# wolfecameron/GIST

Hardware: AMD Instinct MI355X
Metric: epochs/sec (higher is better)
Workload: dtype f32 (projection products from 3 bf16 pieces per operand = all 24 bits, 6 cross terms, fp32 accumulation)

## Files before the change

### gist_amd/_lib.py

```python
import ctypes
import os

_HERE = os.path.dirname(os.path.abspath(__file__))
LIB_PATH = os.environ.get('GIST_LIB_PATH') or os.path.join(_HERE, 'libgist_hip.so')

ABI_VERSION = 16


class GistLibraryError(RuntimeError):
    pass


class GistError(RuntimeError):
    """A gist_* entry point returned a negative code."""


_p = ctypes.c_void_p
_i64 = ctypes.c_int64
_i32 = ctypes.c_int32
_int = ctypes.c_int
_f = ctypes.c_float
_u64 = ctypes.c_uint64

SIGNATURES = {
    'gist_last_error': (ctypes.c_char_p, []),
    'gist_abi_version': (_int, []),
    'gist_device_count': (_int, []),
    'gist_in_degree_norm_f32': (_int, [_p, _i64, _p, _p]),
    'gist_spmm_csr_f32': (_int, [_p, _p, _p, _i64, _p, _i64, _i64, _i64, _p, _p, _int, _p]),
    'gist_partition_last_stats': (_int, [_p, _i32]),
    'gist_partition_graph': (_int, [_p, _p, _p, _p, _i64, _i32, _u64, _i32, _f, _p]),
    'gist_spmm_csr_blocked_f32': (_int, [_p, _p, _p, _i64, _p, _i64, _i64, _i64, _p, _p, _int, _p, _i64, _p]),
    'gist_spmm_blocks_bytes': (_i64, [_i64]),
    'gist_spmm_blocks_prepare': (_int, [_p, _p, _i64, _p, _i64, _p, _i64, _p]),
    'gist_spmm_csr_prepared_f32': (_int, [_p, _p, _p, _i64, _p, _i64, _i64, _i64, _p, _p, _int, _p, _i64, _p, _p]),
    'gist_gemm_workspace_bytes': (_i64, [_i64, _i64, _i64]),
    'gist_gemm_set_mode': (_int, [_int]),
    'gist_gemm_get_mode': (_int, []),
    'gist_tuning_set': (_int, [_int, ctypes.c_double]),
    'gist_tuning_get': (ctypes.c_double, [_int]),
    'gist_launch_count': (ctypes.c_uint64, []),
    'gist_empty_launches': (_int, [ctypes.c_int32, ctypes.c_int32, ctypes.c_int32, _p]),
    'gist_gemm_nt_f32': (_int, [_p, _i64, _p, _i64, _p, _p, _i64, _i64, _i64, _i64, _p, _i64, _p]),
    'gist_gemm_nn_f32': (_int, [_p, _i64, _p, _i64, _p, _i64, _i64, _i64, _i64, _p, _i64, _p]),
    'gist_gemm_tn_f32': (_int, [_p, _i64, _p, _i64, _p, _i64, _i64, _i64, _i64, _p, _i64, _p]),
    'gist_ln_relu_fwd_f32': (_int, [_p, _i64, _p, _i64, _p, _i64, _i64, _int, _int, _f, _p]),
    'gist_ln_relu_bwd_f32': (_int, [_p, _i64, _p, _i64, _p, _p, _i64, _i64, _i64, _int, _int, _p]),
    'gist_gemm_nn_dropout_f32': (_int, [_p, _i64, _p, _i64, _p, _i64, _i64, _i64, _i64, _f, _u64, _u64, _p, _i64, _p]),
    'gist_dropout_f32': (_int, [_p, _i64, _i64, _i64, _f, _u64, _u64, _p]),
    'gist_colsum_partials': (_i64, [_i64]),
    'gist_colsum_f32': (_int, [_p, _i64, _i64, _i64, _p, _p, _p]),
    'gist_softmax_xent_f32': (_int, [_p, _i64, _p, _p, _i64, _p, _p, _p, _i64, _i64, _i64, _p]),
    'gist_adam_f32': (_int, [_p, _p, _p, _p, _i64, _f, _f, _f, _f, _f, _i64, _p]),
    'gist_argmax_correct_i32': (_int, [_p, _i64, _p, _p, _p, _i64, _i64, _p]),
    'gist_induced_mark': (_int, [_p, _i64, _p, _p]),
    'gist_induced_unmark': (_int, [_p, _i64, _p, _p]),
    'gist_fill_i32': (_int, [_p, _i64, _i32, _p]),
    'gist_copy_i32': (_int, [_p, _p, _i64, _p]),
    'gist_publish_i64': (_int, [_p, _i64, _p, _p]),
    'gist_induced_rowptr': (_int, [_p, _p, _p, _i64, _p, _p, _p]),
    'gist_induced_fill': (_int, [_p, _p, _p, _i64, _p, _p, _p, _i64, _p]),
    'gist_extract_batch': (_int, [_p, _p, _p, _p, _p, _i64, _p, _p, _p, _p, _p, _i64, _p, _p, _i64, _i64, _p, _i64, _p, _p, _p]),
    'gist_gather_rows_f32': (_int, [_p, _i64, _p, _i64, _i64, _p, _i64, _p]),
    'gist_gather_i32': (_int, [_p, _p, _i64, _p, _p]),
    'gist_block_gather_f32': (_int, [_p, _i64, _p, _p, _i64, _i64, _p, _i64, _p]),
    'gist_block_scatter_f32': (_int, [_p, _i64, _p, _p, _i64, _i64, _p, _i64, _p]),
    'gist_mean_rows_f32': (_int, [_p, _i64, _i64, _i64, _p, _p]),
    'gist_standard_scaler_workspace_bytes': (_i64, [_i64, _i64]),
    'gist_standard_scaler_f32': (_int, [_p, _i64, _i64, _i64, _p, _i64, _p, _p, _p, _i64, _p]),
    'gist_timer_create': (_p, [_i64]),
    'gist_timer_destroy': (None, [_p]),
    'gist_timer_reset': (None, [_p]),
    'gist_timer_count': (_i64, [_p]),
    'gist_timer_read': (_int, [_p, _i64, _p, _p, _p, _p, _p]),
    'gist_step_h3_workspace_bytes': (_i64, [_p]),
    'gist_step_h3_workspace_bytes_mode': (_i64, [_p, _int]),
    'gist_step_fused_workspace_bytes': (_i64, [_p]),
    'gist_step_col_partials_floats': (_i64, [_p]),
    'gist_step_fused_slab_bytes': (_i64, [_p, _i32]),
    'gist_spmm_csr_drop_f32': (_int, [_p, _p, _p, _i64, _p, _i64, _i64, _i64, _p, _p, _int, _p, _i64, _int, _f,
                                      _u64, _u64, _u64, _i64, _p]),
    'gist_spmm_csr_drop_prepared_f32': (_int, [_p, _p, _p, _i64, _p, _i64, _i64, _i64, _p, _p, _int, _p, _i64, _int, _f,
                                               _u64, _u64, _u64, _i64, _p, _p]),
    'gist_spmm_csr_drop_lnbwd_f32': (_int, [_p, _p, _p, _i64, _p, _i64, _i64, _i64, _p, _p, _i64, _f, _u64, _u64, _u64, _i64,
                                            _p, _i64, _p, _p, _i64, _p, _i64, _int, _p]),
    'gist_spmm_lnb_units': (_i64, [_i64]),
    'gist_spmm_block_image_bytes': (_i64, []),
    'gist_spmm_pair_min_edges': (ctypes.c_int32, []),
    'gist_spmm_block_units_f32': (_int, [_p, _i64, _p, _p, _i64, _p, _i64, _i64, _i64, _p, _int, _p]),
    'gist_spmm_block_chains_f32': (_int, [_p, _i64, _p, _p, _p, _i64, _p, _i64, _i64, _i64, _p, _int, _p]),
    'gist_spmm_prepared_useful': (_int, [_i64, _i64, _i64, _p, _p]),
    'gist_spmm_drop_takes': (_int, [_int, _i64, _i64, _i64, _p, _p, _int]),
    'gist_gemm_dual_takes': (_int, [_i64, _i64, _i64, _i64, _i64, _i64, _i64, _p, _p, _p, _p]),
    'gist_gemm_nn_tn_dual_f32': (_int, [_p, _i64, _p, _i64, _p, _i64, _p, _i64, _p, _i64, _i64, _i64, _i64, _p, _i64, _p, _p]),
    'gist_gemm_slabs_f32': (_int, [_int, _p, _i64, _p, _i64, _p, _p, _i64, _i64, _i64, _i64, _p, _i64, _p, _p]),
    'gist_ln_relu_fwd_drop_f32': (_int, [_p, _i64, _p, _i64, _p, _i64, _p, _i64, _i64, _int, _int, _f, _f, _u64,
                                         _u64, _i64, _p]),
    'gist_ln_relu_fwd_slabs_f32': (_int, [_p, _i64, _p, _i64, _int, _p, _p, _i64, _p, _i64, _p, _i64, _i64, _int, _int,
                                          _f, _f, _u64, _u64, _i64, _p]),
    'gist_gemm_splits_operands': (_int, [_i64, _i64, _i64]),
    'gist_row_chunks16': (_i64, [_i64]),
    'gist_ln_relu_bwd_colsum_f32': (_int, [_p, _i64, _p, _i64, _p, _p, _i64, _i64, _i64, _int, _int, _p, _p]),
    'gist_colsum_chunks_f32': (_int, [_p, _i64, _i64, _p, _p]),
    'gist_class_layer_takes': (_int, [_i64, _i64, _i64, _i64, _i64, _p, _p]),
    'gist_class_layer_f32': (_int, [_p, _i64, _p, _i64, _p, _p, _i64, _p, _i64, _p, _i64, _p, _p, _i64, _f, _u64, _u64,
                                    _p, _i64, _i64, _i64, _p]),
    'gist_class_dw_slab_bytes': (_i64, [_i64, _i64, _i64]),
    'gist_class_dw_slabs_f32': (_int, [_p, _i64, _p, _i64, _p, _i64, _p, _i64, _i64, _i64, _p]),
    'gist_ln_relu_bwd_colsum_class_dw_f32': (_int, [_p, _i64, _p, _i64, _p, _p, _i64, _i64, _i64, _int, _int, _p,
                                                    _p, _i64, _p, _i64, _p, _i64, _p, _i64, _i64, _i64, _p]),
    'gist_gemm_nn_dropout_colsum_f32': (_int, [_p, _i64, _p, _i64, _p, _i64, _i64, _i64, _i64, _f, _u64, _u64,
                                               _p, _i64, _p, _p]),
    'gist_softmax_xent_slabs_f32': (_int, [_p, _i64, _p, _i64, _i64, _p, _p, _p, _i64, _p, _p, _p, _i64, _i64,
                                           _i64, _p]),
    'gist_adam_segments_f32': (_int, [_p, _p, _p, _p, _i64, _f, _f, _f, _f, _f, _i64, _p, _i64, _p, _i64, _i64,
                                      _p, _p]),
    'gist_grad_segments_finish_f32': (_int, [_p, _i64, _p, _i64, _p]),
    'gist_extract_batch_drop': (_int, [_p, _p, _p, _p, _p, _i64, _p, _p, _p, _p, _p, _i64, _p, _p, _i64, _i64, _p,
                                       _i64, _p, _p, _p, _i64, _f, _u64, _u64, _i64, _p]),
    'gist_extract_parts_scratch_bytes': (_i64, [_i64]),
    'gist_extract_parts_supported': (_int, [_i64]),
    'gist_extract_parts_batch': (_int, [_p, _p, _p, _p, _p, _i64, _i64, _p, _p, _i32, _p, _p, _p, _p, _i64,
                                        _p, _p, _i64, _i64, _p, _i64, _p, _p, _p, _i64, _f, _u64, _u64, _i64, _p,
                                        _p]),
    'gist_sage_step': (_int, [_p, _p, _i64, _u64, _f, _f, _f, _f, _f, _i64, _int, _p]),
    'gist_sage_step_extracts_next': (_int, [_p, _i64, _int]),
    'gist_extract_parts_desc_batch': (_int, [_p, _p]),
    'gist_adam_segments_extract_f32': (_int, [_p, _p, _p, _p, _i64, _f, _f, _f, _f, _f, _i64, _p, _i64, _p, _i64, _i64,
                                              _p, _p, _p]),
}

GIST_MAX_LAYERS = 16
TUNE = {'h3_min_gflop': 0, 'h3_min_tiles': 1, 'h3_tm': 2, 'gemm_tile': 3, 'gemm_splits': 4,
        'spmm_chunk': 5, 'spmm_split': 6, 'spmm_kernel': 7, 'b3c': 8, 'class_fused': 9, 'gemm_dual': 10, 'host_threads': 11, 'lnb_fused': 12, 'b3c_splits': 13, 'b3_tail': 14}
GIST_STEP_EXTRACT = 1
GIST_STEP_TRAIN = 2
GIST_STEP_EXTRACT_NEXT = 4
GIST_STEP_PREEXTRACTED = 8
GIST_STEP_PHASE_FORWARD = 16
GIST_STEP_PHASE_BACKWARD = 32
GIST_STEP_PHASE_OPTIMIZER = 64
GIST_STEP_DLOGITS_GIVEN = 128


class LayerDesc(ctypes.Structure):
    _fields_ = [('n_in', _i64), ('n_out', _i64), ('W', _p), ('b', _p), ('dW', _p), ('db', _p),
                ('Z', _p), ('ldz', _i64), ('Y', _p), ('ldy', _i64), ('rstd', _p)]


class StepPlan(ctypes.Structure):
    _fields_ = [('n_layers', _i32), ('use_layernorm', _i32), ('p_drop', _f), ('seed', _u64),
                ('layer', LayerDesc * GIST_MAX_LAYERS),
                ('dlogits', _p), ('ldc', _i64), ('dZ', _p), ('partials', _p),
                ('row_loss', _p), ('loss', _p), ('workspace', _p), ('workspace_bytes', _i64),
                ('workspace2', _p), ('workspace2_bytes', _i64),
                ('params', _p), ('grads', _p), ('exp_avg', _p), ('exp_avg_sq', _p),
                ('n_params', _i64),
                ('g_rowptr', _p), ('g_col', _p), ('g_t_rowptr', _p), ('g_t_col', _p),
                ('feat', _p), ('ld_feat', _i64), ('labels_all', _p), ('remap', _p),
                ('rowptr', _p), ('col', _p), ('t_rowptr', _p), ('t_col', _p),
                ('col_capacity', _i64), ('norm', _p), ('labels', _p), ('timer', _p),
                ('n_max', _i64), ('feat_absmax', _f), ('h3_workspace', _p),
                ('h3_workspace_bytes', _i64), ('row_blocks', _p), ('n_row_blocks', _i64),
                ('spmm_prepared', _p), ('spmm_prepared_bytes', _i64),
                ('fuse', _i32), ('hsrc', _p * GIST_MAX_LAYERS), ('ld_hsrc', _i64 * GIST_MAX_LAYERS),
                ('col_partials', _p), ('fused_workspace', _p), ('fused_workspace_bytes', _i64),
                ('node_part', _p), ('part_slot', _p),
                ('batch_index', _i32), ('extract_scratch', _p),
                ('next_ids', _p), ('next_n', _i64), ('next_batch_index', _i32), ('next_drop_offset', _u64),
                ('feat_intra', _p), ('ld_feat_intra', _i64), ('sibling_parts', ctypes.c_int32)]


class ExtractPartsDesc(ctypes.Structure):
    _fields_ = [('g_rowptr', _p), ('g_col', _p), ('g_t_rowptr', _p), ('g_t_col', _p),
                ('ids', _p), ('n', _i64), ('n_max', _i64),
                ('node_part', _p), ('part_slot', _p), ('batch', _i32),
                ('rowptr', _p), ('col', _p), ('t_rowptr', _p), ('t_col', _p), ('col_capacity', _i64), ('norm', _p),
                ('feat', _p), ('ld_feat', _i64), ('n_feat', _i64), ('z0', _p), ('ldz0', _i64),
                ('labels_all', _p), ('labels', _p),
                ('x0', _p), ('ldx0', _i64), ('p', _f), ('seed', _u64), ('offset', _u64), ('mask_ld', _i64),
                ('scratch', _p), ('feat_intra', _p), ('ld_intra', _i64), ('ah', _p)]


class GradSegment(ctypes.Structure):
    _fields_ = [('begin', _i64), ('end', _i64), ('src', _p), ('stride', _i64), ('n_src', _i32)]


_lib = None


def load():
    global _lib
    if _lib is not None:
        return _lib
    if not os.path.exists(LIB_PATH):
        raise GistLibraryError(
            'gist_amd: %s is missing. Build it with `python gist_amd/build.py` '
            '(hipcc --offload-arch=gfx950). There is no CPU fallback.' % LIB_PATH)
    import torch
    try:
        lib = ctypes.CDLL(LIB_PATH)
    except OSError as e:
        raise GistLibraryError('gist_amd: cannot load %s: %s' % (LIB_PATH, e))
    for name, (res, args) in SIGNATURES.items():
        try:
            fn = getattr(lib, name)
        except AttributeError:
            raise GistLibraryError('gist_amd: %s does not export %s (stale build?)'
                                   % (LIB_PATH, name))
        fn.restype = res
        fn.argtypes = args
    if lib.gist_abi_version() != ABI_VERSION:
        raise GistLibraryError('gist_amd: ABI version mismatch: library %d, binding %d'
                               % (lib.gist_abi_version(), ABI_VERSION))
    _lib = lib
    return lib


def check(rc, name):
    if rc != 0:
        msg = load().gist_last_error()
        raise GistError('%s failed (%d): %s' % (name, rc, msg.decode() if msg else ''))
```

### gist_amd/csrc/gemm_b3.hip

```cpp
#include <stdlib.h>
#include <string.h>

#include <type_traits>

#include "common.h"

namespace gist {

typedef __bf16 bf16x8 __attribute__((ext_vector_type(8)));
typedef float b3_f32x4 __attribute__((ext_vector_type(4)));

constexpr int B3_TM = 256, B3_TN = 128, B3_BK = 32;
constexpr int B3_THREADS = 512;
constexpr int B3_STAGES = 2;
constexpr int B3_SKEW = 16;
constexpr int B3_KT_BYTES = B3_BK * 6;
constexpr int B3_A_BYTES = B3_TM * B3_KT_BYTES;
constexpr int B3_B_BYTES = B3_TN * B3_KT_BYTES;
constexpr int B3_BUF_BYTES = B3_A_BYTES + B3_B_BYTES;

__device__ __forceinline__ uint32_t b3_pack(__bf16 lo, __bf16 hi) {
    return (uint32_t)__builtin_bit_cast(unsigned short, lo) |
           ((uint32_t)__builtin_bit_cast(unsigned short, hi) << 16);
}
// ... 159 lines not shown
    b3_f32x4 acc[NI][NJ];
#pragma unroll
    for (int i = 0; i < NI; ++i)
#pragma unroll
        for (int j = 0; j < NJ; ++j)
#pragma unroll
            for (int e = 0; e < 4; ++e) acc[i][j][e] = 0.f;

    constexpr int NWAVES = B3_THREADS / 64;
    constexpr int DA = B3_TM / 16 * 3 / NWAVES, DB = B3_TN / 16 * 3 / NWAVES;
    uint32_t offA[DA], offB[DB];
    b3_dma_offsets<DA>(g.lda, g.m, row0, DA * wave, lane, offA);
    b3_dma_offsets<DB>(g.ldb, g.n, col0, DB * wave, lane, offB);
    const char *originA = reinterpret_cast<const char *>(g.a) + (int64_t)row0 * g.lda * 6 + (int64_t)kt0 * B3_KT_BYTES;
    const char *originB = reinterpret_cast<const char *>(g.b) + (int64_t)col0 * g.ldb * 6 + (int64_t)kt0 * B3_KT_BYTES;
    auto dma = [&](int buf, int kt) {
        char *sa = b3_smem + buf * B3_BUF_BYTES;
        b3_dma_image<DA>(originA + (int64_t)kt * B3_KT_BYTES, offA, sa, DA * wave);
        b3_dma_image<DB>(originB + (int64_t)kt * B3_KT_BYTES, offB, sa + B3_A_BYTES, DB * wave);
    };

    const char *fa[B3_STAGES][3], *fb[B3_STAGES][3];
#pragma unroll
    for (int p = 0; p < 3; ++p) {
        const int c = 3 * kg + p;
        const int in_slab = (rr * 12 + (c ^ ((rr >> 3) << 1))) * 16;
#pragma unroll
        for (int st = 0; st < B3_STAGES; ++st) {
            fa[st][p] = b3_smem + st * B3_BUF_BYTES + wm * NI * 3072 + in_slab;
            fb[st][p] = b3_smem + st * B3_BUF_BYTES + B3_A_BYTES + wn * NJ * 3072 + in_slab;
        }
    }

    const bool live = __builtin_amdgcn_readfirstlane(row0 + wm * (16 * NI) < g.m);
    bf16x8 a[NI][3], b[NJ][3];
    auto read_head = [&](auto st_c) {
        constexpr int st = decltype(st_c)::value;
        if (!live) return;
#pragma unroll
        for (int j = 0; j < NJ; ++j) b[j][0] = *reinterpret_cast<const bf16x8 *>(fb[st][0] + j * 3072);
#pragma unroll
        for (int i = 0; i < NI; ++i) a[i][1] = *reinterpret_cast<const bf16x8 *>(fa[st][1] + i * 3072);
#pragma unroll
        for (int i = 0; i < NI; ++i) a[i][2] = *reinterpret_cast<const bf16x8 *>(fa[st][2] + i * 3072);
    };
    auto read_rest = [&](auto st_c) {
        constexpr int st = decltype(st_c)::value;
        if (!live) return;
#pragma unroll
        for (int j = 0; j < NJ; ++j) b[j][1] = *reinterpret_cast<const bf16x8 *>(fb[st][1] + j * 3072);
#pragma unroll
        for (int i = 0; i < NI; ++i) a[i][0] = *reinterpret_cast<const bf16x8 *>(fa[st][0] + i * 3072);
#pragma unroll
        for (int j = 0; j < NJ; ++j) b[j][2] = *reinterpret_cast<const bf16x8 *>(fb[st][2] + j * 3072);
    };
    constexpr int pa[6] = {1, 2, 1, 0, 0, 0};
    constexpr int pb[6] = {0, 0, 1, 0, 1, 2};
    constexpr int B3_MID = 4 * NI * NJ;

    dma(0, 0);
    __builtin_amdgcn_s_waitcnt(0x0f70);
    __syncthreads();
    dma(1, 1);
    read_head(std::integral_constant<int, 0>{});

    auto mfmas = [&](auto t0_c, auto t1_c) {
        constexpr int t0 = decltype(t0_c)::value, t1 = decltype(t1_c)::value;
        if (!live) return;
#pragma unroll
        for (int t = t0; t < t1; ++t) {
            const int term = t / (NI * NJ), i = (t % (NI * NJ)) / NJ, j = t % NJ;
            b3_mfma(acc[i][j], a[i][pa[term]], b[j][pb[term]]);
        }
    };
    const int last_kt = n_kt - 1;
    auto kstep = [&](auto cur_c, auto late_c, int kt) {
        constexpr int cur = decltype(cur_c)::value;
        constexpr int skew = decltype(late_c)::value * B3_SKEW;
        using I = std::integral_constant<int, 0>;
        __builtin_amdgcn_sched_barrier(0);
        __builtin_amdgcn_s_setprio(1);
        mfmas(I{}, std::integral_constant<int, skew>{});
        __builtin_amdgcn_sched_barrier(0);
        read_rest(cur_c);
        __builtin_amdgcn_sched_barrier(0);
        mfmas(std::integral_constant<int, skew>{}, std::integral_constant<int, B3_MID>{});
        __builtin_amdgcn_sched_barrier(0);
        __builtin_amdgcn_s_waitcnt(0x0070);
        __syncthreads();
        mfmas(std::integral_constant<int, B3_MID>{}, std::integral_constant<int, B3_MID + skew>{});
        __builtin_amdgcn_sched_barrier(0);
        dma(cur, min(kt + 2, last_kt));
        read_head(std::integral_constant<int, cur ^ 1>{});
        __builtin_amdgcn_sched_barrier(0);
        mfmas(std::integral_constant<int, B3_MID + skew>{}, std::integral_constant<int, 6 * NI * NJ>{});
        __builtin_amdgcn_s_setprio(0);
        __builtin_amdgcn_sched_barrier(0);
    };
    auto run = [&](auto late_c) {
        using C0 = std::integral_constant<int, 0>;
        using C1 = std::integral_constant<int, 1>;
        for (int kt = 0; kt < n_kt; kt += 2) {
            kstep(C0{}, late_c, kt);
            kstep(C1{}, late_c, kt + 1);
        }
    };
    if (wave >= 4) run(std::integral_constant<int, 1>{});
    else run(std::integral_constant<int, 0>{});
    __builtin_amdgcn_s_waitcnt(0x0070);

    asm volatile("s_nop 15\n\ts_nop 15" ::: "memory");
    const int rows_valid = min(g.m - row0, B3_TM);
    if (tail) {
        const bool rows_live = wm * (16 * NI) < rows_valid;
        b3_f32x4 *mine = reinterpret_cast<b3_f32x4 *>(g.tail_partials) +
                         (int64_t)(tail_tile * g.tail_splits + tail_slice) * (NI * NJ * B3_THREADS) + threadIdx.x;
        if (rows_live) {
#pragma unroll
            for (int i = 0; i < NI; ++i)
#pragma unroll
                for (int j = 0; j < NJ; ++j) mine[(i * NJ + j) * B3_THREADS] = acc[i][j];
        }
        return;
    }
    float *cbase = g.c + (int64_t)blockIdx.y * g.split_stride + (int64_t)row0 * g.ldc + col0;
    __amdgpu_buffer_rsrc_t crsrc = __builtin_amdgcn_make_buffer_rsrc(
        cbase, 0, (int)((int64_t)rows_valid * g.ldc * 4), 0x00020000);
    const uint32_t ldc_b = (uint32_t)g.ldc * 4;
    uint32_t cvoff[NJ];
    float bv[NJ];
#pragma unroll
    for (int j = 0; j < NJ; ++j) {
        const int cl = wn * (16 * NJ) + j * 16 + rr;
        const bool ok = col0 + cl < g.n;
        cvoff[j] = ok ? (uint32_t)(wm * (16 * NI) + 4 * kg) * ldc_b + (uint32_t)cl * 4 : 0x7fffffffu;
        bv[j] = (g.bias != nullptr && ok) ? g.bias[col0 + cl] : 0.f;
    }
#pragma unroll
    for (int i = 0; i < NI; ++i)
#pragma unroll
        for (int e = 0; e < 4; ++e) {
            const uint32_t roff = (uint32_t)(i * 16 + e) * ldc_b;
#pragma unroll
            for (int j = 0; j < NJ; ++j) {
                const float v = acc[i][j][e] + bv[j];
                if (rows_valid == B3_TM)
                    __builtin_amdgcn_raw_buffer_store_b32(__float_as_uint(v), crsrc, cvoff[j], roff, 0);
                else
                    __builtin_amdgcn_raw_buffer_store_b32(__float_as_uint(v), crsrc, cvoff[j] + roff, 0, 0);
            }
        }
}

__global__ __launch_bounds__(B3_THREADS) void gemm_b3_tail_sum_kernel(B3Args g) {
    constexpr int NI = 4, NJ = 4, GM = 8;
    const int L = g.dp_tiles + (int)blockIdx.x;
    const int width = GM * g.tiles_n;
    const int first_m = (L / width) * GM;
    const int gsz = min(g.tiles_m - first_m, GM);
    const int row0 = (first_m + (L % width) % gsz) * B3_TM, col0 = ((L % width) / gsz) * B3_TN;
    const int lane = threadIdx.x & 63, wave = threadIdx.x >> 6;
    const int wm = wave >> 1, wn = wave & 1, rr = lane & 15, kg = lane >> 4;
    const int reg = blockIdx.y, i = reg / NJ, j = reg % NJ;
    const int row = row0 + wm * (16 * NI) + i * 16 + 4 * kg, col = col0 + wn * (16 * NJ) + j * 16 + rr;
    if (row0 + wm * (16 * NI) >= g.m || col >= g.n) return;
    const b3_f32x4 *part = reinterpret_cast<const b3_f32x4 *>(g.tail_partials) +
                           ((int64_t)blockIdx.x * g.tail_splits * (NI * NJ) + reg) * B3_THREADS + threadIdx.x;
    b3_f32x4 sum = part[0];
    for (int q = 1; q < g.tail_splits; ++q) sum += part[(int64_t)q * (NI * NJ) * B3_THREADS];
    const float bv = g.bias != nullptr ? g.bias[col] : 0.f;
#pragma unroll
    for (int e = 0; e < 4; ++e)
        if (row + e < g.m) g.c[(int64_t)(row + e) * g.ldc + col] = sum[e] + bv;
}

int64_t b3_kpad(int64_t k) { return ceil_div(k, 2 * B3_BK) * (2 * B3_BK); }

int b3_splits(int64_t m, int64_t n, int64_t k) {
    const int64_t tiles = ceil_div(m, B3_TM) * ceil_div(n, B3_TN);
    const int64_t n_kt = b3_kpad(k) / B3_BK;
    const int forced = (int)tune(GIST_TUNE_GEMM_SPLITS);
    int64_t s = forced > 0 ? forced : (tiles >= 192 ? 1 : 256 / tiles);
    if (forced <= 0 && tiles > 128 && tiles < 192) {
        int64_t best = n_kt + 4;
        for (int64_t c = 2; c <= 4; ++c) {
            const int64_t per = ceil_div(ceil_div(n_kt, c), 2) * 2;
            const int64_t cost = ceil_div(tiles * c, 256) * per + 8;
            if (per >= 8 && cost < best) { best = cost; s = c; }
        }
    }
    if (forced <= 0 && s > n_kt / 8) s = n_kt / 8;
    if (s > n_kt / 2) s = n_kt / 2;
    if (s < 1) s = 1;
    const int64_t per = ceil_div(ceil_div(n_kt, s), 2) * 2;
    return (int)ceil_div(n_kt, per);
}
struct B3Tail { int dp_tiles, splits, kt; };
constexpr int B3_CUS = 256;
static B3Tail b3_tail(int64_t m, int64_t n, int64_t k) {
    const int64_t tiles = ceil_div(m, B3_TM) * ceil_div(n, B3_TN);
    B3Tail t{(int)tiles, 1, 0};
    if (tune(GIST_TUNE_B3_TAIL) == 1.0 || tiles <= B3_CUS) return t;
    const int64_t r = tiles % B3_CUS;
    if (r == 0 || r > B3_CUS / 2) return t;
    const int64_t n_kt = b3_kpad(k) / B3_BK;
    int64_t s = B3_CUS / r;
    if (s > n_kt / 8) s = n_kt / 8;
    if (s < 2) return t;
    const int64_t per = ceil_div(ceil_div(n_kt, s), 2) * 2;
    s = ceil_div(n_kt, per);
    if (s < 2) return t;
    t.dp_tiles = (int)(tiles - r); t.splits = (int)s; t.kt = (int)per;
    return t;
}
static int64_t b3_tail_bytes(int64_t m, int64_t n, int64_t k) {
    const B3Tail t = b3_tail(m, n, k);
    if (t.splits < 2) return 0;
    const int64_t r = ceil_div(m, B3_TM) * ceil_div(n, B3_TN) - t.dp_tiles;
    return r * t.splits * (int64_t)(B3_TM * B3_TN * 4);
}
int64_t b3_slab_bytes(int64_t m, int64_t n, int64_t k) {
    const int s = b3_splits(m, n, k);
    return s > 1 ? (int64_t)s * m * n * 4 : b3_tail_bytes(m, n, k);
}

static bool b3_shape_ok(int64_t m, int64_t n, int64_t k, double default_min_gflop) {
    const double t_gflop = tune(GIST_TUNE_H3_MIN_GFLOP), t_tiles = tune(GIST_TUNE_H3_MIN_TILES);
    const double min_gflop = t_gflop > 0.0 ? t_gflop : default_min_gflop;
    const int min_wgs = t_tiles > 0.0 ? (int)t_tiles : 128;
    if (t_tiles <= 0.0 && (m < 64 || n < 64 || k < 64)) return false;
    if (m < 1 || n < 1 || k < 1) return false;
    const int64_t tiles = ceil_div(m, B3_TM) * ceil_div(n, B3_TN);
    if (tiles * b3_splits(m, n, k) < min_wgs) return false;
    if (t_tiles <= 0.0 && (double)m * (double)n < 0.6 * (double)(tiles * B3_TM * B3_TN)) return false;
    if (2.0 * (double)m * (double)n * (double)k < min_gflop * 1e9) return false;
    if (b3_kpad(k) * 6 >= (1LL << 23)) return false;
    return true;
}
bool b3_eligible(int64_t m, int64_t n, int64_t k) { return h3_mode() == 2 && b3_shape_ok(m, n, k, 16.0); }
bool b3_eligible_kept(int64_t m, int64_t n, int64_t k) { return b3_shape_ok(m, n, k, 9.0); }

static int64_t b3_operand_bytes(int64_t m, int64_t n, int64_t k) {
    return ceil_div((m + n) * b3_kpad(k) * 6 + 512, 256) * 256;
}
int64_t b3_workspace_bytes(int64_t m, int64_t n, int64_t k) {
    if (!b3_eligible(m, n, k)) return 0;
    return b3_operand_bytes(m, n, k) + b3_slab_bytes(m, n, k);
}

int b3_dual_split(const B3Dual &d, hipStream_t st) {
    if (d.rows <= 0 || d.cols <= 0) return GIST_OK;
    const int64_t ldd_r = b3_kpad(d.cols), ldd_t = b3_kpad(d.rows);
    const int64_t gx = ceil_div(d.dst_r ? ldd_r : d.cols, 64), gy = ceil_div(d.dst_t ? ldd_t : d.rows, 64);
    B3Dual dd = d;
    dd.vec4 = aligned16(d.src) && d.ld % 4 == 0;
    hipLaunchKernelGGL(b3_dual_split_kernel, dim3((unsigned)gx, (unsigned)gy), dim3(256), 0, st, dd, ldd_r,
                       ldd_t, d.p > 0.f ? 1.0f / (1.0f - d.p) : 1.0f);
    return launch_status("b3_dual_split");
}

int b3_gemm_presplit(const char *name, const uint16_t *sa, const uint16_t *sb, const float *bias, float *c,
                     int64_t ldc, int64_t m, int64_t n, int64_t k, float *slabs, int64_t slab_bytes,
                     hipStream_t st, int *deferred) {
    static DeviceOnce once;
    int dev;
    if (once.needed(&dev)) {
        hipError_t e = hipFuncSetAttribute(reinterpret_cast<const void *>(&gemm_b3_kernel),
                                           hipFuncAttributeMaxDynamicSharedMemorySize, B3_STAGES * B3_BUF_BYTES);
        if (e != hipSuccess) {
            set_error("%s: hipFuncSetAttribute: %s", name, hipGetErrorString(e));
            return GIST_ELAUNCH;
        }
        once.done(dev);
    }
    if (ldc * B3_TM * 4 >= (1LL << 31)) {
        set_error("%s: leading dimension of the output >= 2^21 elements on the bf16x3 path", name);
        return GIST_EINVAL;
    }
    B3Args g;
    const int64_t kpad = b3_kpad(k);
    g.a = sa; g.lda = kpad; g.b = sb; g.ldb = kpad; g.bias = bias; g.c = c; g.ldc = ldc;
    g.m = (int)m; g.n = (int)n; g.kpad = (int)kpad;
    g.tiles_m = (int)ceil_div(m, B3_TM);
    g.tiles_n = (int)ceil_div(n, B3_TN);
    const int64_t n_kt = kpad / B3_BK;
    int splits = b3_splits(m, n, k);
    if (splits > 1 && (slabs == nullptr || slab_bytes < (int64_t)splits * m * n * 4)) splits = 1;
    g.kt_per_split = (int)(ceil_div(ceil_div(n_kt, splits), 2) * 2);
    splits = (int)ceil_div(n_kt, g.kt_per_split);
    g.split_stride = 0;
    if (splits > 1) { g.c = slabs; g.ldc = n; g.split_stride = m * n; g.bias = nullptr; }
    g.dp_tiles = g.tiles_m * g.tiles_n; g.tail_splits = 1; g.tail_kt = 0;
    g.tail_partials = nullptr;
    unsigned grid_x = (unsigned)g.dp_tiles;
    if (splits == 1 && slabs != nullptr && aligned16(slabs)) {
        const B3Tail t = b3_tail(m, n, k);
        if (t.splits > 1 && slab_bytes >= b3_tail_bytes(m, n, k)) {
            const int r = g.dp_tiles - t.dp_tiles;
            g.dp_tiles = t.dp_tiles; g.tail_splits = t.splits; g.tail_kt = t.kt;
            g.tail_partials = slabs;
            grid_x = (unsigned)(t.dp_tiles + r * t.splits);
        }
    }
    const int64_t slot = timer_begin(tl_timer, 2, m, n, k, st);
    hipLaunchKernelGGL(gemm_b3_kernel, dim3(grid_x, (unsigned)splits),
                       dim3(B3_THREADS), B3_STAGES * B3_BUF_BYTES, st, g);
    int rc = launch_status(name);
    if (rc == GIST_OK && g.tail_splits > 1) {
        hipLaunchKernelGGL(gemm_b3_tail_sum_kernel, dim3((grid_x - (unsigned)g.dp_tiles) / (unsigned)g.tail_splits, 16),
                           dim3(B3_THREADS), 0, st, g);
        rc = launch_status(name);
    }
    if (deferred) *deferred = splits;
    else if (rc == GIST_OK && splits > 1) rc = splitk_reduce(name, slabs, m * n, splits, bias, c, ldc, m, n, st);
    timer_end(tl_timer, slot, st);
    return rc;
}

int b3_gemm(const char *name, bool a_kc, bool b_kc, const float *a, int64_t lda, const float *b,
            int64_t ldb, const float *bias, float *c, int64_t ldc, int64_t m, int64_t n, int64_t k,
            void *ws, int64_t ws_bytes, hipStream_t st) {
    if (!b3_eligible(m, n, k)) return 0;
    if (ldc * B3_TM * 4 >= (1LL << 31)) return 0;
    if (ws == nullptr || !aligned16(ws) || ws_bytes < b3_workspace_bytes(m, n, k)) return 0;
    const int64_t kpad = b3_kpad(k);
    uint16_t *sa = static_cast<uint16_t *>(ws);
    uint16_t *sb = sa + m * kpad * 3;
    float *slabs = reinterpret_cast<float *>(static_cast<char *>(ws) + b3_operand_bytes(m, n, k));
    auto split = [&](bool kc, const float *src, int64_t ld, int64_t rows, uint16_t *dst) {
        B3Dual d{};
        d.src = src; d.ld = ld;
        if (kc) { d.rows = rows; d.cols = k; d.dst_r = dst; }
        else { d.rows = k; d.cols = rows; d.dst_t = dst; }
        return b3_dual_split(d, st);
    };
    int rc = split(a_kc, a, lda, m, sa);
    if (rc != GIST_OK) return rc;
    rc = split(b_kc, b, ldb, n, sb);
    if (rc != GIST_OK) return rc;
    rc = b3_gemm_presplit(name, sa, sb, bias, c, ldc, m, n, k, slabs, b3_slab_bytes(m, n, k), st, nullptr);
    return rc == GIST_OK ? 1 : rc;
}

}
```

### include/gist_hip.h

```cpp
#ifndef GIST_HIP_H_
#define GIST_HIP_H_

#include <stdint.h>

#ifdef __cplusplus
extern "C" {
#endif

typedef void *gist_stream_t;

#define GIST_OK 0
#define GIST_EINVAL (-1)
#define GIST_ELAUNCH (-2)
#define GIST_ENOSPACE (-3)

const char *gist_last_error(void);
int gist_abi_version(void);
int gist_device_count(void);


int gist_in_degree_norm_f32(const int32_t *rowptr, int64_t n_rows, float *norm,
                            gist_stream_t stream);

int gist_spmm_csr_f32(const int32_t *rowptr, const int32_t *col,
                      const float *x, int64_t ldx, float *y, int64_t ldy,
                      int64_t n_rows, int64_t d,
                      const float *out_scale, const float *src_scale,
                      int accumulate, gist_stream_t stream);

int gist_spmm_csr_blocked_f32(const int32_t *rowptr, const int32_t *col,
                              const float *x, int64_t ldx, float *y, int64_t ldy,
                              int64_t n_rows, int64_t d,
                              const float *out_scale, const float *src_scale, int accumulate,
                              const int32_t *row_blocks, int64_t n_row_blocks,
                              gist_stream_t stream);

int64_t gist_spmm_blocks_bytes(int64_t n_row_blocks);
int gist_spmm_blocks_prepare(const int32_t *rowptr, const int32_t *col, int64_t n_rows,
                             const int32_t *row_blocks, int64_t n_row_blocks,
                             void *prepared, int64_t prepared_bytes, gist_stream_t stream);
int gist_spmm_csr_prepared_f32(const int32_t *rowptr, const int32_t *col,
                               const float *x, int64_t ldx, float *y, int64_t ldy,
                               int64_t n_rows, int64_t d,
                               const float *out_scale, const float *src_scale, int accumulate,
                               const int32_t *row_blocks, int64_t n_row_blocks,
                               const void *prepared, gist_stream_t stream);

int gist_spmm_csr_drop_f32(const int32_t *rowptr, const int32_t *col,
                           const float *x, int64_t ldx, float *y, int64_t ldy,
                           int64_t n_rows, int64_t d,
                           const float *out_scale, const float *src_scale, int accumulate,
                           const int32_t *row_blocks, int64_t n_row_blocks,
                           int mode, float p, uint64_t seed, uint64_t y_offset, uint64_t src_offset,
                           int64_t mask_ld, gist_stream_t stream);
int gist_spmm_drop_takes(int mode, int64_t d, int64_t ldx, int64_t ldy, const float *x, const float *y,
                         int has_row_blocks);
int gist_spmm_csr_drop_prepared_f32(const int32_t *rowptr, const int32_t *col,
                                    const float *x, int64_t ldx, float *y, int64_t ldy,
                                    int64_t n_rows, int64_t d,
                                    const float *out_scale, const float *src_scale, int accumulate,
                                    const int32_t *row_blocks, int64_t n_row_blocks,
                                    int mode, float p, uint64_t seed, uint64_t y_offset, uint64_t src_offset,
                                    int64_t mask_ld, const void *prepared, gist_stream_t stream);
int gist_spmm_csr_drop_lnbwd_f32(const int32_t *rowptr, const int32_t *col, const float *x, int64_t ldx, const float *y,
                                 int64_t ldy, int64_t n_rows, int64_t d, const float *src_scale, const int32_t *row_blocks,
                                 int64_t n_row_blocks, float p, uint64_t seed, uint64_t y_offset, uint64_t src_offset,
                                 int64_t mask_ld, const float *yhat, int64_t ldyh, const float *rstd, float *dy, int64_t lddy,
                                 float *col_partials, int64_t partial_rows, int relu, gist_stream_t stream);
int64_t gist_spmm_lnb_units(int64_t n_row_blocks);

int gist_spmm_prepared_useful(int64_t d, int64_t ldx, int64_t ldy, const float *x, const float *y);

int64_t gist_spmm_block_image_bytes(void);
int32_t gist_spmm_pair_min_edges(void);
int gist_spmm_block_units_f32(const int32_t *units, int64_t n_units, const void *images, const float *x, int64_t ldx,
                              float *y, int64_t ldy, int64_t n_rows_y, int64_t d, const float *out_scale,
                              int accumulate, gist_stream_t stream);
int gist_spmm_block_chains_f32(const int32_t *chain_ptr, int64_t n_chains, const int32_t *units, const void *images,
                               const float *x, int64_t ldx, float *y, int64_t ldy, int64_t n_rows_y, int64_t d,
                               const float *out_scale, int accumulate, gist_stream_t stream);


int gist_partition_graph(const int32_t *rowptr, const int32_t *col,
                         const int32_t *t_rowptr, const int32_t *t_col, int64_t n, int32_t k,
                         uint64_t seed, int32_t n_passes, float imbalance, int32_t *part);
int gist_partition_last_stats(double *out, int32_t n);


int64_t gist_gemm_workspace_bytes(int64_t m, int64_t n, int64_t k);
int gist_gemm_splits_operands(int64_t m, int64_t n, int64_t k);

int gist_gemm_nt_f32(const float *a, int64_t lda, const float *w, int64_t ldw,
                     const float *bias, float *y, int64_t ldy,
                     int64_t m, int64_t n, int64_t k,
                     void *workspace, int64_t workspace_bytes, gist_stream_t stream);

int gist_gemm_nn_f32(const float *g, int64_t ldg, const float *w, int64_t ldw,
                     float *z, int64_t ldz, int64_t m, int64_t n, int64_t k,
                     void *workspace, int64_t workspace_bytes, gist_stream_t stream);

int gist_gemm_tn_f32(const float *g, int64_t ldg, const float *a, int64_t lda,
                     float *d, int64_t ldd, int64_t m, int64_t n, int64_t k,
                     void *workspace, int64_t workspace_bytes, gist_stream_t stream);

int gist_gemm_slabs_f32(int layout, const float *a, int64_t lda, const float *b, int64_t ldb,
                        const float *bias, float *c, int64_t ldc, int64_t m, int64_t n, int64_t k,
                        void *slabs, int64_t slab_bytes, int32_t *n_slabs, gist_stream_t stream);

int gist_gemm_set_mode(int mode);
int gist_gemm_get_mode(void);

#define GIST_TUNE_H3_MIN_GFLOP 0
#define GIST_TUNE_H3_MIN_TILES 1
#define GIST_TUNE_H3_TM 2
#define GIST_TUNE_GEMM_TILE 3
#define GIST_TUNE_GEMM_SPLITS 4
#define GIST_TUNE_SPMM_CHUNK 5
#define GIST_TUNE_SPMM_SPLIT 6
#define GIST_TUNE_SPMM_KERNEL 7
#define GIST_TUNE_B3C 8
#define GIST_TUNE_CLASS_FUSED 9
#define GIST_TUNE_GEMM_DUAL 10
#define GIST_TUNE_HOST_THREADS 11
#define GIST_TUNE_LNB_FUSED 12
#define GIST_TUNE_B3C_SPLITS 13
#define GIST_TUNE_B3_TAIL 14
#define GIST_TUNE_COUNT 15
int gist_tuning_set(int knob, double value);
double gist_tuning_get(int knob);

uint64_t gist_launch_count(void);
int gist_empty_launches(int32_t n, int32_t grid, int32_t block, gist_stream_t stream);


int gist_ln_relu_fwd_f32(float *y, int64_t ldy, float *out, int64_t ldo,
                         float *rstd, int64_t n_rows, int64_t d,
                         int use_lynorm, int relu, float eps, gist_stream_t stream);

int gist_ln_relu_fwd_drop_f32(float *y, int64_t ldy, float *out, int64_t ldo, float *out2, int64_t ldo2,
                              float *rstd, int64_t n_rows, int64_t d, int use_lynorm, int relu,
                              float eps, float p, uint64_t seed, uint64_t offset, int64_t mask_ld,
                              gist_stream_t stream);

int gist_ln_relu_fwd_slabs_f32(float *y, int64_t ldy, const float *slabs, int64_t slab_stride,
                               int32_t n_slabs, const float *bias, float *out, int64_t ldo, float *out2,
                               int64_t ldo2, float *rstd, int64_t n_rows, int64_t d, int use_lynorm,
                               int relu, float eps, float p, uint64_t seed, uint64_t offset,
                               int64_t mask_ld, gist_stream_t stream);

int64_t gist_row_chunks16(int64_t n_rows);
int gist_ln_relu_bwd_colsum_f32(const float *d_out, int64_t ldg, const float *yhat, int64_t ldy,
                                const float *rstd, float *dy, int64_t lddy, int64_t n_rows, int64_t d,
                                int use_lynorm, int relu, float *col_partials, gist_stream_t stream);
int gist_ln_relu_bwd_colsum_class_dw_f32(const float *d_out, int64_t ldg, const float *yhat, int64_t ldy,
                                         const float *rstd, float *dy, int64_t lddy, int64_t n_rows, int64_t d,
                                         int use_lynorm, int relu, float *col_partials,
                                         const float *d_logits, int64_t ld_dlogits, const float *z, int64_t ldz,
                                         float *slabs, int64_t slab_bytes, int32_t *n_slabs, int64_t n_rows_cls,
                                         int64_t n_classes, int64_t k, gist_stream_t stream);
int gist_colsum_chunks_f32(const float *partials, int64_t chunks, int64_t d, float *out,
                           gist_stream_t stream);

int gist_ln_relu_bwd_f32(const float *d_out, int64_t ldg, const float *yhat, int64_t ldy,
                         const float *rstd, float *dy, int64_t lddy,
                         int64_t n_rows, int64_t d, int use_lynorm, int relu,
                         gist_stream_t stream);

int gist_dropout_f32(float *z, int64_t ldz, int64_t n_rows, int64_t d, float p,
                     uint64_t seed, uint64_t offset, gist_stream_t stream);

int gist_gemm_nn_dropout_f32(const float *g, int64_t ldg, const float *w, int64_t ldw,
                             float *z, int64_t ldz, int64_t m, int64_t n, int64_t k,
                             float p, uint64_t seed, uint64_t offset,
                             void *workspace, int64_t workspace_bytes, gist_stream_t stream);

int gist_gemm_nn_dropout_colsum_f32(const float *g, int64_t ldg, const float *w, int64_t ldw,
                                    float *z, int64_t ldz, int64_t m, int64_t n, int64_t k,
                                    float p, uint64_t seed, uint64_t offset,
                                    void *workspace, int64_t workspace_bytes, float *g_col_partials,
                                    gist_stream_t stream);

int gist_class_layer_takes(int64_t n_rows, int64_t n_classes, int64_t k, int64_t ldz, int64_t ldw,
                           const float *z, const float *w);
int gist_class_layer_f32(const float *z, int64_t ldz, const float *w, int64_t ldw, const float *bias,
                         const int32_t *labels, int64_t count, float *logits, int64_t ldl,
                         float *d_logits, int64_t ldg, float *row_loss, float *dz, int64_t lddz,
                         float p, uint64_t seed, uint64_t offset, float *dlogits_col_partials,
                         int64_t n_rows, int64_t n_classes, int64_t k, gist_stream_t stream);
int64_t gist_class_dw_slab_bytes(int64_t n_rows, int64_t n_classes, int64_t k);
int gist_class_dw_slabs_f32(const float *d_logits, int64_t ldg, const float *z, int64_t ldz,
                            float *slabs, int64_t slab_bytes, int32_t *n_slabs, int64_t n_rows,
                            int64_t n_classes, int64_t k, gist_stream_t stream);

int gist_gemm_dual_takes(int64_t m, int64_t n, int64_t k, int64_t lddy, int64_t ldw, int64_t ldz, int64_t lddz,
                         const float *dy, const float *w, const float *z, const float *dz);
int gist_gemm_nn_tn_dual_f32(const float *dy, int64_t lddy, const float *w, int64_t ldw, float *dz, int64_t lddz,
                             const float *z, int64_t ldz, float *dw, int64_t lddw, int64_t m, int64_t n, int64_t k,
                             void *slabs, int64_t slab_bytes, int32_t *n_slabs, gist_stream_t stream);

int64_t gist_colsum_partials(int64_t n_rows);
int gist_colsum_f32(const float *g, int64_t ldg, int64_t n_rows, int64_t d,
                    float *partials, float *out, gist_stream_t stream);


int gist_softmax_xent_f32(const float *logits, int64_t ldl, const int32_t *labels,
                          const uint8_t *mask, int64_t count, float *row_loss,
                          float *loss, float *d_logits, int64_t ldg, int64_t n_rows,
                          int64_t n_classes, gist_stream_t stream);

int gist_softmax_xent_slabs_f32(float *logits, int64_t ldl, const float *slabs, int64_t slab_stride,
                                int64_t n_slabs, const float *bias, const int32_t *labels,
                                const uint8_t *mask, int64_t count, float *row_loss, float *loss,
                                float *d_logits, int64_t ldg, int64_t n_rows, int64_t n_classes,
                                gist_stream_t stream);

int gist_adam_f32(float *param, const float *grad, float *exp_avg, float *exp_avg_sq,
                  int64_t n, float lr, float beta1, float beta2, float eps,
                  float weight_decay, int64_t step, gist_stream_t stream);

typedef struct gist_grad_segment {
    int64_t begin, end;
    const float *src;
    int64_t stride;
    int32_t n_src;
} gist_grad_segment;
int gist_adam_segments_f32(float *param, float *grad, float *exp_avg, float *exp_avg_sq,
                           int64_t n, float lr, float beta1, float beta2, float eps,
                           float weight_decay, int64_t step,
                           const gist_grad_segment *segments, int64_t n_segments,
                           const float *row_loss, int64_t n_loss_rows, int64_t loss_count, float *loss,
                           gist_stream_t stream);

int gist_grad_segments_finish_f32(float *grad, int64_t n, const gist_grad_segment *segments, int64_t n_segments,
                                  gist_stream_t stream);

int gist_argmax_correct_i32(const float *logits, int64_t ldl, const int32_t *labels,
                            const uint8_t *mask, int32_t *correct, int64_t n_rows,
                            int64_t n_classes, gist_stream_t stream);


int gist_induced_mark(const int32_t *ids, int64_t n_ids, int32_t *remap, gist_stream_t stream);
int gist_induced_unmark(const int32_t *ids, int64_t n_ids, int32_t *remap, gist_stream_t stream);
int gist_fill_i32(int32_t *p, int64_t n, int32_t value, gist_stream_t stream);

int gist_copy_i32(const int32_t *src, int32_t *dst, int64_t n, gist_stream_t stream);
int gist_publish_i64(const int64_t *device_word, int64_t tag, int64_t *host_word, gist_stream_t stream);

int gist_induced_rowptr(const int32_t *rowptr, const int32_t *col, const int32_t *ids,
                        int64_t n_ids, const int32_t *remap, int32_t *sub_rowptr,
                        gist_stream_t stream);

int gist_induced_fill(const int32_t *rowptr, const int32_t *col, const int32_t *ids,
                      int64_t n_ids, const int32_t *remap, const int32_t *sub_rowptr,
                      int32_t *sub_col, int64_t sub_col_capacity, gist_stream_t stream);

int gist_extract_batch(const int32_t *g_rowptr, const int32_t *g_col,
                       const int32_t *g_t_rowptr, const int32_t *g_t_col,
                       const int32_t *ids, int64_t n, int32_t *remap,
                       int32_t *rowptr, int32_t *col, int32_t *t_rowptr, int32_t *t_col,
                       int64_t col_capacity, float *norm,
                       const float *feat, int64_t ld_feat, int64_t n_feat,
                       float *z0, int64_t ldz0,
                       const int32_t *labels_all, int32_t *labels, gist_stream_t stream);

int gist_extract_batch_drop(const int32_t *g_rowptr, const int32_t *g_col,
                            const int32_t *g_t_rowptr, const int32_t *g_t_col,
                            const int32_t *ids, int64_t n, int32_t *remap,
                            int32_t *rowptr, int32_t *col, int32_t *t_rowptr, int32_t *t_col,
                            int64_t col_capacity, float *norm,
                            const float *feat, int64_t ld_feat, int64_t n_feat,
                            float *z0, int64_t ldz0,
                            const int32_t *labels_all, int32_t *labels,
                            float *x0, int64_t ldx0, float p, uint64_t seed, uint64_t offset,
                            int64_t mask_ld, gist_stream_t stream);

int64_t gist_extract_parts_scratch_bytes(int64_t n_max);
int gist_extract_parts_supported(int64_t n_max);
int gist_extract_parts_batch(const int32_t *g_rowptr, const int32_t *g_col,
                             const int32_t *g_t_rowptr, const int32_t *g_t_col,
                             const int32_t *ids, int64_t n, int64_t n_max,
// ... 139 lines not shown
```

Before: 5.136.

## Add 256x256-tile bf16x3 GEMM kernel with single-buffered A and double-buffered B

Result: faster. 5.306, median of 6 (+3.3%).

```diff
diff --git a/gist_amd/_lib.py b/gist_amd/_lib.py
--- a/gist_amd/_lib.py
+++ b/gist_amd/_lib.py
@@ -132,7 +132,8 @@
 
 GIST_MAX_LAYERS = 16
 TUNE = {'h3_min_gflop': 0, 'h3_min_tiles': 1, 'h3_tm': 2, 'gemm_tile': 3, 'gemm_splits': 4,
-        'spmm_chunk': 5, 'spmm_split': 6, 'spmm_kernel': 7, 'b3c': 8, 'class_fused': 9, 'gemm_dual': 10, 'host_threads': 11, 'lnb_fused': 12, 'b3c_splits': 13, 'b3_tail': 14}
+        'spmm_chunk': 5, 'spmm_split': 6, 'spmm_kernel': 7, 'b3c': 8, 'class_fused': 9, 'gemm_dual': 10, 'host_threads': 11, 'lnb_fused': 12, 'b3c_splits': 13, 'b3_tail': 14,
+        'b3_wide': 15}
 GIST_STEP_EXTRACT = 1
 GIST_STEP_TRAIN = 2
 GIST_STEP_EXTRACT_NEXT = 4
diff --git a/gist_amd/csrc/gemm_b3.hip b/gist_amd/csrc/gemm_b3.hip
--- a/gist_amd/csrc/gemm_b3.hip
+++ b/gist_amd/csrc/gemm_b3.hip
@@ -335,6 +335,186 @@
         }
 }
 
+constexpr int B3W_TN = 256;
+constexpr int B3W_B_BYTES = B3W_TN * B3_KT_BYTES;
+constexpr int B3W_LDS_BYTES = B3_A_BYTES + 2 * B3W_B_BYTES;
+
+__global__ __launch_bounds__(B3_THREADS, 1) void gemm_b3_wide_kernel(B3Args g) {
+    extern __shared__ __attribute__((aligned(16))) char b3_smem[];
+    constexpr int NI = 4, NJ = 8;
+    const int nwg = g.dp_tiles;
+    const int orig = blockIdx.x;
+    const int qd = nwg / kXcds, rm = nwg % kXcds, xcd = orig % kXcds;
+    const int L = (xcd < rm ? xcd * (qd + 1) : rm * (qd + 1) + (xcd - rm) * qd) + orig / kXcds;
+    constexpr int GM = 8;
+    const int width = GM * g.tiles_n;
+    const int group = L / width;
+    const int first_m = group * GM;
+    const int gsz = min(g.tiles_m - first_m, GM);
+    const int bm = first_m + (L % width) % gsz;
+    const int bn = (L % width) / gsz;
+    const int row0 = bm * B3_TM, col0 = bn * B3W_TN;
+    const int n_kt = g.kpad / B3_BK;
+
+    const int lane = threadIdx.x & 63;
+    const int wave = __builtin_amdgcn_readfirstlane(threadIdx.x >> 6);
+    const int wm = wave >> 1, wn = wave & 1;
+    const int rr = lane & 15, kg = lane >> 4;
+
+    b3_f32x4 acc[NI][NJ];
+#pragma unroll
+    for (int i = 0; i < NI; ++i)
+#pragma unroll
+        for (int j = 0; j < NJ; ++j)
+#pragma unroll
+            for (int e = 0; e < 4; ++e) acc[i][j][e] = 0.f;
+
+    constexpr int NWAVES = B3_THREADS / 64;
+    constexpr int DA = B3_TM / 16 * 3 / NWAVES, DB = B3W_TN / 16 * 3 / NWAVES;
+    uint32_t offA[DA], offB[DB];
+    b3_dma_offsets<DA>(g.lda, g.m, row0, DA * wave, lane, offA);
+    b3_dma_offsets<DB>(g.ldb, g.n, col0, DB * wave, lane, offB);
+    const char *originA = reinterpret_cast<const char *>(g.a) + (int64_t)row0 * g.lda * 6;
+    const char *originB = reinterpret_cast<const char *>(g.b) + (int64_t)col0 * g.ldb * 6;
+    auto dma = [&](int bbuf, int kt) {
+        b3_dma_image<DA>(originA + (int64_t)kt * B3_KT_BYTES, offA, b3_smem, DA * wave);
+        b3_dma_image<DB>(originB + (int64_t)kt * B3_KT_BYTES, offB, b3_smem + B3_A_BYTES + bbuf * B3W_B_BYTES,
+                         DB * wave);
+    };
+
+    const char *fa[3], *fb[2][3];
+#pragma unroll
+    for (int p = 0; p < 3; ++p) {
+        const int c = 3 * kg + p;
+        const int in_slab = (rr * 12 + (c ^ ((rr >> 3) << 1))) * 16;
+        fa[p] = b3_smem + wm * NI * 3072 + in_slab;
+#pragma unroll
+        for (int st = 0; st < 2; ++st) fb[st][p] = b3_smem + B3_A_BYTES + st * B3W_B_BYTES + wn * NJ * 3072 + in_slab;
+    }
+
+    auto body = [&](auto live_c) {
+        constexpr bool live = decltype(live_c)::value;
+        bf16x8 a[NI][3], b[2][3];
+        auto read_a = [&](auto p_c) {
+            constexpr int p = decltype(p_c)::value;
+            if constexpr (!live) return;
+#pragma unroll
+            for (int i = 0; i < NI; ++i) a[i][p] = *reinterpret_cast<const bf16x8 *>(fa[p] + i * 3072);
+        };
+        auto read_b = [&](auto st_c, auto pair_c, auto p_c) {
+            constexpr int st = decltype(st_c)::value, pair = decltype(pair_c)::value, p = decltype(p_c)::value;
+            if constexpr (!live) return;
+#pragma unroll
+            for (int jj = 0; jj < 2; ++jj) b[jj][p] = *reinterpret_cast<const bf16x8 *>(fb[st][p] + (2 * pair + jj) * 3072);
+        };
+        constexpr int pa[6] = {1, 2, 1, 0, 0, 0};
+        constexpr int pb[6] = {0, 0, 1, 0, 1, 2};
+        auto mfmas = [&](auto pair_c, auto t0_c, auto t1_c) {
+            constexpr int pair = decltype(pair_c)::value, t0 = decltype(t0_c)::value, t1 = decltype(t1_c)::value;
+            if constexpr (!live) return;
+#pragma unroll
+            for (int term = t0; term < t1; ++term)
+#pragma unroll
+                for (int jj = 0; jj < 2; ++jj)
+#pragma unroll
+                    for (int i = 0; i < NI; ++i) b3_mfma(acc[i][2 * pair + jj], a[i][pa[term]], b[jj][pb[term]]);
+        };
+        using I0 = std::integral_constant<int, 0>;
+        using I1 = std::integral_constant<int, 1>;
+        using I2 = std::integral_constant<int, 2>;
+        using I3 = std::integral_constant<int, 3>;
+
+        dma(0, 0);
+        __builtin_amdgcn_s_waitcnt(0x0f70);
+        __syncthreads();
+        read_a(I1{}); read_a(I2{});
+        read_b(I0{}, I0{}, I0{}); read_b(I0{}, I0{}, I1{}); read_b(I0{}, I0{}, I2{});
+        read_a(I0{});
+        __builtin_amdgcn_s_waitcnt(0xc07f);
+
+        const int last_kt = n_kt - 1;
+        auto kstep = [&](auto cur_c, int kt) {
+            constexpr int cur = decltype(cur_c)::value;
+            auto pair_block = [&](auto pair_c) {
+                constexpr int pair = decltype(pair_c)::value;
+                using S = std::integral_constant<int, pair < 3 ? cur : (cur ^ 1)>;
+                using P = std::integral_constant<int, pair < 3 ? pair + 1 : 0>;
+                __builtin_amdgcn_sched_barrier(0);
+                mfmas(pair_c, I0{}, I3{});
+                __builtin_amdgcn_sched_barrier(0);
+                if constexpr (pair == 0) {
+                    __builtin_amdgcn_s_waitcnt(0xc07f);
+                    __syncthreads();
+                    dma(cur ^ 1, min(kt + 1, last_kt));
+                }
+                if constexpr (pair == 3) {
+                    __builtin_amdgcn_s_waitcnt(0x0070);
+                    __syncthreads();
+                    read_a(I1{}); read_a(I2{});
+                }
+                __builtin_amdgcn_sched_barrier(0);
+                mfmas(pair_c, I3{}, std::integral_constant<int, 4>{});
+                __builtin_amdgcn_sched_barrier(0);
+                read_b(S{}, P{}, I0{});
+                __builtin_amdgcn_sched_barrier(0);
+                mfmas(pair_c, std::integral_constant<int, 4>{}, std::integral_constant<int, 5>{});
+                if constexpr (pair == 3) __builtin_amdgcn_s_waitcnt(0xc27f);
+                __builtin_amdgcn_sched_barrier(0);
+                read_b(S{}, P{}, I1{});
+                __builtin_amdgcn_sched_barrier(0);
+                mfmas(pair_c, std::integral_constant<int, 5>{}, std::integral_constant<int, 6>{});
+                __builtin_amdgcn_sched_barrier(0);
+                read_b(S{}, P{}, I2{});
+                if constexpr (pair == 3) read_a(I0{});
+            };
+            __builtin_amdgcn_s_setprio(1);
+            pair_block(I0{});
+            pair_block(I1{});
+            pair_block(I2{});
+            pair_block(I3{});
+            __builtin_amdgcn_s_setprio(0);
+            __builtin_amdgcn_sched_barrier(0);
+        };
+        for (int kt = 0; kt < n_kt; kt += 2) {
+            kstep(I0{}, kt);
+            kstep(I1{}, kt + 1);
+        }
+    };
+    if (__builtin_amdgcn_readfirstlane(row0 + wm * (16 * NI) < g.m)) body(std::true_type{});
+    else body(std::false_type{});
+    __builtin_amdgcn_s_waitcnt(0x0070);
+
+    asm volatile("s_nop 15\n\ts_nop 15" ::: "memory");
+    const int rows_valid = min(g.m - row0, B3_TM);
+    float *cbase = g.c + (int64_t)row0 * g.ldc + col0;
+    __amdgpu_buffer_rsrc_t crsrc = __builtin_amdgcn_make_buffer_rsrc(
+        cbase, 0, (int)((int64_t)rows_valid * g.ldc * 4), 0x00020000);
+    const uint32_t ldc_b = (uint32_t)g.ldc * 4;
+    uint32_t cvoff[NJ];
+    float bv[NJ];
+#pragma unroll
+    for (int j = 0; j < NJ; ++j) {
+        const int cl = wn * (16 * NJ) + j * 16 + rr;
+        const bool ok = col0 + cl < g.n;
+        cvoff[j] = ok ? (uint32_t)(wm * (16 * NI) + 4 * kg) * ldc_b + (uint32_t)cl * 4 : 0x7fffffffu;
+        bv[j] = (g.bias != nullptr && ok) ? g.bias[col0 + cl] : 0.f;
+    }
+#pragma unroll
+    for (int i = 0; i < NI; ++i)
+#pragma unroll
+        for (int e = 0; e < 4; ++e) {
+            const uint32_t roff = (uint32_t)(i * 16 + e) * ldc_b;
+#pragma unroll
+            for (int j = 0; j < NJ; ++j) {
+                const float v = acc[i][j][e] + bv[j];
+                if (rows_valid == B3_TM)
+                    __builtin_amdgcn_raw_buffer_store_b32(__float_as_uint(v), crsrc, cvoff[j], roff, 0);
+                else
+                    __builtin_amdgcn_raw_buffer_store_b32(__float_as_uint(v), crsrc, cvoff[j] + roff, 0, 0);
+            }
+        }
+}
+
 __global__ __launch_bounds__(B3_THREADS) void gemm_b3_tail_sum_kernel(B3Args g) {
     constexpr int NI = 4, NJ = 4, GM = 8;
     const int L = g.dp_tiles + (int)blockIdx.x;
@@ -402,6 +582,11 @@
     const int64_t r = ceil_div(m, B3_TM) * ceil_div(n, B3_TN) - t.dp_tiles;
     return r * t.splits * (int64_t)(B3_TM * B3_TN * 4);
 }
+static bool b3_wide(int64_t m, int64_t n, int64_t k) {
+    if (tune(GIST_TUNE_B3_WIDE) == 1.0) return false;
+    if (ceil_div(m, B3_TM) * ceil_div(n, B3W_TN) < B3_CUS) return false;
+    return b3_splits(m, n, k) == 1 && b3_tail(m, n, k).splits < 2;
+}
 int64_t b3_slab_bytes(int64_t m, int64_t n, int64_t k) {
     const int s = b3_splits(m, n, k);
     return s > 1 ? (int64_t)s * m * n * 4 : b3_tail_bytes(m, n, k);
@@ -450,6 +635,9 @@
     if (once.needed(&dev)) {
         hipError_t e = hipFuncSetAttribute(reinterpret_cast<const void *>(&gemm_b3_kernel),
                                            hipFuncAttributeMaxDynamicSharedMemorySize, B3_STAGES * B3_BUF_BYTES);
+        if (e == hipSuccess)
+            e = hipFuncSetAttribute(reinterpret_cast<const void *>(&gemm_b3_wide_kernel),
+                                    hipFuncAttributeMaxDynamicSharedMemorySize, B3W_LDS_BYTES);
         if (e != hipSuccess) {
             set_error("%s: hipFuncSetAttribute: %s", name, hipGetErrorString(e));
             return GIST_ELAUNCH;
@@ -486,6 +674,15 @@
         }
     }
     const int64_t slot = timer_begin(tl_timer, 2, m, n, k, st);
+    if (b3_wide(m, n, k) && splits == 1 && g.tail_splits == 1) {
+        g.tiles_n = (int)ceil_div(n, B3W_TN);
+        g.dp_tiles = g.tiles_m * g.tiles_n;
+        hipLaunchKernelGGL(gemm_b3_wide_kernel, dim3((unsigned)g.dp_tiles), dim3(B3_THREADS), B3W_LDS_BYTES, st, g);
+        const int rc = launch_status(name);
+        if (deferred) *deferred = 1;
+        timer_end(tl_timer, slot, st);
+        return rc;
+    }
     hipLaunchKernelGGL(gemm_b3_kernel, dim3(grid_x, (unsigned)splits),
                        dim3(B3_THREADS), B3_STAGES * B3_BUF_BYTES, st, g);
     int rc = launch_status(name);
diff --git a/include/gist_hip.h b/include/gist_hip.h
--- a/include/gist_hip.h
+++ b/include/gist_hip.h
@@ -125,7 +125,8 @@
 #define GIST_TUNE_LNB_FUSED 12
 #define GIST_TUNE_B3C_SPLITS 13
 #define GIST_TUNE_B3_TAIL 14
-#define GIST_TUNE_COUNT 15
+#define GIST_TUNE_B3_WIDE 15
+#define GIST_TUNE_COUNT 16
 int gist_tuning_set(int knob, double value);
 double gist_tuning_get(int knob);
 
```
